# esologic/GANce

Measured on AMD Instinct MI355X. Metric: synthesized frames/sec at 1024x1024 config-f, higher is better.
Workload: dtype f32 (bf16x3 split operands, 6 terms, fp32 accumulate)

## Files before the change

### gance_amd/csrc/engine.hip

```cpp

#include <hip/hip_runtime.h>

#include <algorithm>
#include <cmath>
#include <cstdio>
#include <cstdlib>
#include <cstring>
#include <map>
#include <memory>
#include <mutex>
#include <string>
#include <tuple>
#include <vector>

#include "../../include/gance_hip.h"
#include "kernels.h"

namespace {

thread_local std::string g_last_error;

int fail(int code, const std::string& message) {
    g_last_error = message;
    return code;
// ... 218 lines not shown
    std::vector<size_t> wino64_w;
    float* noise_rand = nullptr;
    std::vector<size_t> noise_rand_off;
    int noise_rand_count = 0;
    bool noise_randomized = false;
    std::vector<size_t> wino43_w;
    std::vector<size_t> upfir_w;
    std::vector<size_t> upfir16_w;
    std::vector<size_t> winogemm_w;
    std::vector<size_t> upgemm_w;
    size_t up_packed_floats = 0, up_prod_floats = 0;
    int gemm_bf16 = 0;
    std::vector<size_t> upfir16x_w;
    std::vector<size_t> upfirs_w;
    int upfir_split = 1;
    int upfir_split_max_res = 1024;
    int num_cus = 256;
    std::vector<float> conv_ns;
    std::vector<int> conv_s_off, conv_d_off;
    std::vector<size_t> rgb_w, rgb_bias;
    std::vector<int> rgb_s_off;
    int ctot = 0, dtot = 0;
    int* blk_row = nullptr;
    gance::DemodLayer* demod_layers = nullptr;

    std::shared_ptr<gance_workspace> ws;
    std::map<std::tuple<int, int, unsigned, int, int>, GraphEntry> graphs;
    std::vector<int> t_units;
    size_t slab_floats = 0, y_floats = 0, rgb_part_floats = 0;

// ... 290 lines not shown
        if (form.wino43) form.wino64 = false;
        return form;
    };
    enum class UpFused { no, fp32, split };
    auto up_runs_fused = [&](int idx, gance::UpFirArgs* plan) -> UpFused {
        const ConvLayerHost& c = e->convs[idx];
        const int H = (1 << c.res_log2) / 2;
        static const int upfir_env = [] { const char* v = std::getenv("GANCE_TUNE_UPFIR"); return v ? std::atoi(v) : -1; }();
        const int upfir_mode = upfir_env >= 0 ? upfir_env
                                              : ((e->cfg.flags & GANCE_FLAG_SPLIT_UPFIR) ? 0 : ((e->cfg.flags & GANCE_FLAG_FORCE_FUSED_UPFIR) ? 2 : 1));
        if (!c.up || upfir_mode == 0 || (e->upfir_w[idx] == SIZE_MAX && e->upfir16_w[idx] == SIZE_MAX)) return UpFused::no;
        gance::UpFirArgs u{};
        u.Cin = c.cin;
        if (e->upfirs_w[idx] != SIZE_MAX && upfir_mode != 0) {
            gance::upfirs_plan(B, c.cout, H, H, e->num_cus, &u);
            if (e->upfir_split == 2 || (u.total_blocks >= e->num_cus * 9 / 16 && 2 * H <= e->upfir_split_max_res)) {
                if (plan != nullptr) *plan = u;
                return UpFused::split;
            }
            u = gance::UpFirArgs{};
            u.Cin = c.cin;
        }
        if (e->upfir16_w[idx] != SIZE_MAX)
            gance::upfir16_plan(B, c.cout, H, H, e->num_cus, &u);
        else
            gance::upfir_plan(B, c.cout, H, H, e->num_cus, &u);
        const int steps_per_seg = u.rows_per_seg / u.step_rows;
        if (plan != nullptr) *plan = u;
        return (upfir_mode == 2 || (u.total_blocks >= e->num_cus * 3 / 4 && (u.segs == 1 || steps_per_seg >= 4))) ? UpFused::fp32 : UpFused::no;
    };
    static const bool prescale_up = [] { const char* v = std::getenv("GANCE_TUNE_PRESCALE_UP"); return !(v && std::atoi(v) == 0); }();
// ... 386 lines not shown
    if (config->device < 0 || config->device >= device_count)
        return fail(GANCE_ERR_INVALID_ARGUMENT, "device ordinal out of range");
    gance::DeviceGuard guard(config->device);
    GANCE_HIP_CHECK(guard.status());
    int num_cus = 0;
    GANCE_HIP_CHECK(hipDeviceGetAttribute(&num_cus, hipDeviceAttributeMultiprocessorCount, config->device));

    gance_engine* e = new gance_engine();
    {
        const char* v = std::getenv("GANCE_TUNE_GEMM_BF16X6");
        e->gemm_bf16 = v != nullptr && std::atoi(v) != 0 ? 1 : 0;
        const char* const split = std::getenv("GANCE_TUNE_UPFIR_SPLIT");
        e->upfir_split = split != nullptr ? std::max(0, std::min(2, std::atoi(split))) : 1;
        const char* const split_res = std::getenv("GANCE_TUNE_UPFIR_SPLIT_MAXRES");
        if (split_res != nullptr) e->upfir_split_max_res = std::atoi(split_res);
    }
    e->cfg = *config;
    e->num_cus = num_cus > 0 ? num_cus : 256;
    e->res_log2 = res_log2;
    e->num_rows = res_log2 * 2 - 2;
    build_spec(res_log2, &e->convs, &e->rgbs);
    const int nconv = (int)e->convs.size();
    const int nrgb = (int)e->rgbs.size();

    e->conv_s_off.resize(nconv);
    e->conv_d_off.resize(nconv);
    e->rgb_s_off.resize(nrgb);
    int ctot = 0, dtot = 0;
    for (int i = 0; i < nconv; ++i) {
        e->conv_s_off[i] = ctot;
// ... 115 lines not shown
            const int split_mode = c.cout % 256 == 0 ? e->gemm_bf16 : 0;
            e->winogemm_w[i] = reserve(gance::winogemm_weight_floats(c.cin, c.cout) * (split_mode ? 3 : 2) / 2);
            if (split_mode) gance::winogemm_arrange_weights_split(scaled.data(), c.cin, c.cout, &pool[e->winogemm_w[i]]);
            else gance::winogemm_arrange_weights(scaled.data(), c.cin, c.cout, &pool[e->winogemm_w[i]]);
        }
        e->upgemm_w.push_back(SIZE_MAX);
        if (c.up && upgemm_min_columns() > 0 && gance::upgemm_supported(c.cin, c.cout, (1 << c.res_log2) / 2, (1 << c.res_log2) / 2)) {
            std::vector<float> scaled(wn);
            for (size_t j = 0; j < wn; ++j) scaled[j] = src[j] * coef;
            const int split_mode = (9 * c.cout) % 256 == 0 ? e->gemm_bf16 : 0;
            e->upgemm_w[i] = reserve(gance::upgemm_weight_floats(c.cin, c.cout) * (split_mode ? 3 : 2) / 2);
            if (split_mode) gance::upgemm_arrange_weights_split(scaled.data(), c.cin, c.cout, kUpTapWeight, &pool[e->upgemm_w[i]]);
            else gance::upgemm_arrange_weights(scaled.data(), c.cin, c.cout, kUpTapWeight, &pool[e->upgemm_w[i]]);
        }
        e->upfirs_w.push_back(SIZE_MAX);
        if (c.up && e->upfir_split != 0 && upfir16_mode() != 0 && gance::upfirs_supported(c.cin, c.cout, (1 << c.res_log2) / 2, (1 << c.res_log2) / 2)) {
            std::vector<float> scaled(wn);
            for (size_t j = 0; j < wn; ++j) scaled[j] = src[j] * coef;
            e->upfirs_w[i] = reserve(gance::upfirs_weight_floats(c.cin, c.cout));
            gance::upfirs_arrange_weights(scaled.data(), c.cin, c.cout, kUpTapWeight, &pool[e->upfirs_w[i]]);
        }
        e->upfir16x_w.push_back(SIZE_MAX);
        if (c.up && upfir16_mode() != 0 && upfir16x_mode() != 0 && gance::upfir16x_supported(c.cin, c.cout, (1 << c.res_log2) / 2, (1 << c.res_log2) / 2)) {
            std::vector<float> scaled(wn);
            for (size_t j = 0; j < wn; ++j) scaled[j] = src[j] * coef;
            e->upfir16x_w[i] = reserve(gance::upfir16x_weight_floats(c.cin, c.cout));
            gance::upfir16x_arrange_weights(scaled.data(), c.cin, c.cout, kUpTapWeight, &pool[e->upfir16x_w[i]]);
        }
        src += wn;
        demod_layers[i] = {(long long)w2_cursor, e->conv_s_off[i], e->conv_d_off[i], c.cin, c.cout};
        w2_cursor += (size_t)c.cin * c.cout;
// ... 386 lines not shown
```

### gance_amd/csrc/kernels.h

```cpp
#ifndef GANCE_KERNELS_H
#define GANCE_KERNELS_H

#include <hip/hip_runtime.h>
#include <stddef.h>
#include <stdint.h>

#include <mutex>
#include <string>

namespace gance {

class DeviceGuard {
  public:
    explicit DeviceGuard(int device) {
        if (hipGetDevice(&previous_) != hipSuccess) previous_ = -1;
        status_ = (device >= 0 && device != previous_) ? hipSetDevice(device) : hipSuccess;
        switched_ = status_ == hipSuccess && device >= 0 && device != previous_;
    }
    ~DeviceGuard() {
        if (switched_ && previous_ >= 0) (void)hipSetDevice(previous_);
    }
    DeviceGuard(const DeviceGuard&) = delete;
    DeviceGuard& operator=(const DeviceGuard&) = delete;
    hipError_t status() const { return status_; }
// ... 134 lines not shown
size_t upfir_weight_floats(int cin, int cout);
void upfir_arrange_weights(const float* w_in , int cin, int cout, const int* up_tap_weight, float* w_out);
void upfir_plan(int B, int cout, int H, int W, int num_cus, UpFirArgs* args);
hipError_t launch_upfir_fused(const UpFirArgs& args, hipStream_t stream);

bool upfir16_supported(int cin, int cout, int H, int W);
size_t upfir16_weight_floats(int cin, int cout);
void upfir16_arrange_weights(const float* w_in , int cin, int cout, const int* up_tap_weight, float* w_out);
void upfir16_plan(int B, int cout, int H, int W, int num_cus, UpFirArgs* args);
hipError_t launch_upfir16_fused(const UpFirArgs& args, hipStream_t stream);
bool upfir16x_supported(int cin, int cout, int H, int W);
size_t upfir16x_weight_floats(int cin, int cout);
void upfir16x_arrange_weights(const float* w_in , int cin, int cout, const int* up_tap_weight, float* w_out);

bool upfirs_supported(int cin, int cout, int H, int W);
size_t upfirs_weight_floats(int cin, int cout);
void upfirs_arrange_weights(const float* w_in , int cin, int cout, const int* up_tap_weight, float* w_out);
void upfirs_plan(int B, int cout, int H, int W, int num_cus, UpFirArgs* args);
hipError_t launch_upfir_split(const UpFirArgs& args, hipStream_t stream);

struct UpGemmArgs {
    const float* x;
    const float* w;
    const float* s;
    const float* d;
    float* packed;
    float* prod;
    float* t;
    long long x_b_stride, cls_stride, unit_stride;
    int B, Cin, Cout, H, W, s_stride, d_stride;
// ... 100 lines not shown
```

### gance_amd/csrc/upfir_split.hip

```cpp

#include <hip/hip_runtime.h>

#include <algorithm>
#include <cstdlib>
#include <cstring>
#include <type_traits>

#include "kernels.h"

#ifndef GANCE_UPFIRS_ABLATE
#define GANCE_UPFIRS_ABLATE 0
#endif

namespace gance {

namespace {

typedef float f32x4 __attribute__((ext_vector_type(4)));
typedef float f32x2 __attribute__((ext_vector_type(2)));
typedef unsigned u32x4 __attribute__((ext_vector_type(4)));
typedef __bf16 bf16x8 __attribute__((ext_vector_type(8)));
typedef __bf16 bf16x2 __attribute__((ext_vector_type(2)));
typedef __attribute__((address_space(3))) void* lds_ptr_t;

constexpr int kBM = 16;
constexpr int kKC = 32;
constexpr int kSW = 64;
constexpr int kTH = 8;
constexpr int kRows = kTH + 1;
constexpr int kPlanes = 12;
constexpr int kPlaneStride = 80;
constexpr int kSlotUnits = kPlanes * kPlaneStride;
constexpr int kRing = 3;
constexpr int kHaloCols = 4;
constexpr int kHaloUnits = kRows * kHaloCols * kPlanes;
constexpr int kHaloTasks = kRows * kHaloCols * 4;
#ifndef GANCE_UPFIRS_WEAVE
#define GANCE_UPFIRS_WEAVE 2
#endif
#ifndef GANCE_UPFIRS_MIN_SEG_ROWS
#define GANCE_UPFIRS_MIN_SEG_ROWS 16
#endif
#ifndef GANCE_UPFIRS_DEPTH
#define GANCE_UPFIRS_DEPTH 6
#endif
constexpr int kDepth = GANCE_UPFIRS_DEPTH;
constexpr int kCarryRows = 3;
constexpr int kPassCh = 4;
constexpr int kPassRows = 8;
constexpr int kTW = 2 * kSW + 4;
constexpr int kCG = kSW / 2;
constexpr int kRG = 64 / kCG;
constexpr int kFR = kPassRows / kRG;
constexpr int kWin = kFR + 3;
constexpr int kCarryFloats = kBM * kCarryRows * kTW;
constexpr int kStageFloats = kPassCh * kPassRows * kTW;
constexpr int kNzPieces = 2 * kPassRows * 2 * kSW / 256;
constexpr float kSqrt2f = 1.4142135623730951f;
static_assert((2 * kRows) % kDepth == 0 && kDepth + 2 < kRows && kRows % kRing == 0, "ring slots and staging registers rotate with the unrolled rows of a chunk pair");

constexpr size_t kRingBytes = (size_t)kRing * kSlotUnits * 16;
constexpr size_t kHaloBytes = (size_t)2 * kHaloUnits * 16;
constexpr int kWUnits = 27 * 64;
constexpr size_t kWBytes = (size_t)kWUnits * 16;
constexpr size_t lds_bytes(int cin) {
    return kRingBytes + kHaloBytes + kWBytes + sizeof(float) * ((size_t)kStageFloats + kNzPieces * 256 + kCarryFloats + cin + 3 * kBM);
}

__host__ __device__ constexpr int tap_cls(int t) { return t < 4 ? 0 : (t < 6 ? 1 : (t < 8 ? 2 : 3)); }
__host__ __device__ constexpr int tap_dy(int t) { return (t == 2 || t == 3 || t == 5) ? 1 : 0; }
__host__ __device__ constexpr int tap_dx(int t) { return (t == 1 || t == 3 || t == 7) ? 1 : 0; }

__device__ __forceinline__ void lds_barrier() {
    asm volatile("s_waitcnt lgkmcnt(0)" ::: "memory");
    __builtin_amdgcn_s_barrier();
    asm volatile("" ::: "memory");
}

__device__ __forceinline__ int fresh_lane() {
    int l;
    asm volatile("v_mbcnt_lo_u32_b32 %0, -1, 0\n\tv_mbcnt_hi_u32_b32 %0, -1, %0" : "=v"(l));
// ... 17 lines not shown
__device__ __forceinline__ void split_unit(const unsigned (&raw)[8], u32x4 (&part)[3]) {
    unsigned w[3][4];
    if (GANCE_UPFIRS_ABLATE & 1) {
#pragma unroll
        for (int q = 0; q < 3; ++q) part[q] = u32x4{raw[q], raw[q + 1], raw[q + 2], raw[q + 3]};
        return;
    }
#pragma unroll
    for (int e = 0; e < 4; ++e) split_pair(__builtin_bit_cast(float, raw[2 * e]), __builtin_bit_cast(float, raw[2 * e + 1]), w[0][e], w[1][e], w[2][e]);
#pragma unroll
    for (int q = 0; q < 3; ++q) part[q] = u32x4{w[q][0], w[q][1], w[q][2], w[q][3]};
}

}

template <bool kPre, bool kNoise>
__device__ __forceinline__ void upfirs_body(const UpFirArgs& p) {
    extern __shared__ __attribute__((aligned(16))) unsigned char smem_raw[];
    u32x4* const ring = reinterpret_cast<u32x4*>(smem_raw);
    u32x4* const halo = ring + kRing * kSlotUnits;
    u32x4* const w_lds = halo + 2 * kHaloUnits;
    float* const stage = reinterpret_cast<float*>(w_lds + kWUnits);
    float* const nz_lds = stage + kStageFloats;
    float* const carry = nz_lds + kNzPieces * 256;
    float* const s_lds = carry + kCarryFloats;
    float* const d_lds = s_lds + (kPre ? 0 : p.Cin);
    float* const b_lds = d_lds + kBM;
    float* const sn_lds = b_lds + kBM;

    const int tid = threadIdx.x;
    const int wave = __builtin_amdgcn_readfirstlane(tid >> 6);
    const int lane = tid & 63;
    const int n16 = lane & 15, kg = lane >> 4;

    int id;
    {
        const int v = blockIdx.x, nwg = p.total_blocks;
        const int q = nwg >> 3, r = nwg & 7, xcd = v & 7;
        id = (xcd < r ? xcd * (q + 1) : r * (q + 1) + (xcd - r) * q) + (v >> 3);
    }
    const int m_tile = id % p.m_tiles;
    id /= p.m_tiles;
    const int strip = id % p.strips;
    id /= p.strips;
    const int seg = id % p.segs;
    const int b = id / p.segs;
    const int m0 = m_tile * kBM;
    const int X0 = strip * kSW;
    const int H = p.H, W = p.W;
    const int Hp = H + 2, Wp = W + 8;
    const int HpWp4 = Hp * Wp * 4;
    const int chunks = p.Cin / kKC;
    const int steps = H / kTH;
    const int s_begin = seg * (p.rows_per_seg / kTH), s_end = s_begin + p.rows_per_seg / kTH;
    const int s_first = seg > 0 ? s_begin - 1 : s_begin;

    const __amdgpu_buffer_rsrc_t x_rsrc =
        __builtin_amdgcn_make_buffer_rsrc((void*)(p.x + (size_t)b * p.x_b_stride), 0, p.Cin * Hp * Wp * 4, 0x00020000);
    const __amdgpu_buffer_rsrc_t w_rsrc = __builtin_amdgcn_make_buffer_rsrc(
        (void*)(reinterpret_cast<const unsigned char*>(p.w) + (size_t)m_tile * chunks * 27 * 1024), 0, chunks * 27 * 1024, 0x00020000);

    const int st_pair = lane >> 4, st_g = lane & 15;
    u32x4* const ring_w = ring + wave * kPlaneStride + ring_column(4 * st_g + st_pair);
    const int m_pos = 16 * wave + n16;
    const u32x4* const ring_r0 = ring + kg * kPlaneStride + ring_column(m_pos);
    const u32x4* const ring_r1 = ring + kg * kPlaneStride + (m_pos > 0 ? ring_column(m_pos - 1) : kEdgeColumn);
    const bool edge_copy = wave == 3 && lane < kPlanes;
    const int e_unit = lane % kPlanes;
    u32x4* const ring_e = ring + (e_unit >> 2) * 4 * kPlaneStride + (e_unit & 3) * kPlaneStride + (edge_copy ? kEdgeColumn : 66 + wave);
    const u32x4* const halo_e = halo + e_unit;
    const u32x4* const halo_r = halo + ((n16 & 7) * kHaloCols + 2 * (n16 >> 3)) * kPlanes + kg;
    const u32x4* const halo_f = halo + ((kRows - 1) * kHaloCols + 2 * (n16 >> 3)) * kPlanes + kg;
    const int st_voff = (2 * st_pair * Hp * Wp + X0 + 4 + 4 * st_g) * 4;
    unsigned st[kDepth][8];
    auto stage_load = [&](unsigned(&dst)[8], int chunk, int brow, bool in_loop = false) {
        if ((GANCE_UPFIRS_ABLATE & 4) && in_loop) return;
        const int soff = ((chunk * kKC + wave * 8) * Hp + brow) * Wp * 4;
#pragma unroll
        for (int e = 0; e < 2; ++e) {
            const u32x4 q4 = __builtin_amdgcn_raw_buffer_load_b128(x_rsrc, st_voff, soff + e * HpWp4, 0);
#pragma unroll
            for (int c = 0; c < 4; ++c) dst[2 * c + e] = q4[c];
        }
    };
    auto scale_pair = [&](unsigned(&raw)[8], int chunk) {
        if constexpr (!kPre) {
            const f32x2 s2 = *reinterpret_cast<const f32x2*>(s_lds + chunk * kKC + 8 * wave + 2 * st_pair);
#pragma unroll
            for (int c = 0; c < 4; ++c) {
                raw[2 * c] = __builtin_bit_cast(unsigned, __builtin_bit_cast(float, raw[2 * c]) * s2[0]);
                raw[2 * c + 1] = __builtin_bit_cast(unsigned, __builtin_bit_cast(float, raw[2 * c + 1]) * s2[1]);
            }
        }
    };
    auto transpose_rows = [](u32x4& u) {
        auto a02 = __builtin_amdgcn_permlane32_swap(u[0], u[2], false, false);
        auto a13 = __builtin_amdgcn_permlane32_swap(u[1], u[3], false, false);
        auto b01 = __builtin_amdgcn_permlane16_swap(a02[0], a13[0], false, false);
        auto b23 = __builtin_amdgcn_permlane16_swap(a02[1], a13[1], false, false);
        u = u32x4{b01[0], b01[1], b23[0], b23[1]};
    };
    auto scale8 = [&](unsigned(&raw)[8], int chunk, int group) {
        if constexpr (!kPre) {
            const f32x4 s0 = *reinterpret_cast<const f32x4*>(s_lds + chunk * kKC + group * 8);
            const f32x4 s1 = *reinterpret_cast<const f32x4*>(s_lds + chunk * kKC + group * 8 + 4);
#pragma unroll
            for (int e = 0; e < 4; ++e) {
                raw[e] = __builtin_bit_cast(unsigned, __builtin_bit_cast(float, raw[e]) * s0[e]);
                raw[4 + e] = __builtin_bit_cast(unsigned, __builtin_bit_cast(float, raw[4 + e]) * s1[e]);
            }
        }
    };
    auto stage_store = [&](unsigned(&raw)[8], int slot, int chunk) {
        scale_pair(raw, chunk);
        u32x4 part[3];
        split_unit(raw, part);
#pragma unroll
        for (int q = 0; q < 3; ++q) transpose_rows(part[q]);
#pragma unroll
        for (int q = 0; q < 3; ++q)
            if (!(GANCE_UPFIRS_ABLATE & 16)) ring_w[slot * kSlotUnits + q * 4 * kPlaneStride] = part[q];
    };
    auto edge_store = [&](int slot, int hbuf, int hrow) { if (!(GANCE_UPFIRS_ABLATE & 64)) ring_e[slot * kSlotUnits] = halo_e[hbuf * kHaloUnits + (hrow * kHaloCols + 1) * kPlanes]; };
    const int h_task = tid < kHaloTasks ? tid : tid - kHaloTasks;
    const int h_col = h_task & 3, h_kg = (h_task >> 2) & 3, h_row = h_task >> 4;
    const int h_voff = ((h_kg * 8 * Hp + h_row) * Wp + X0 + 2 + (h_col & 1) + (h_col >> 1) * 65) * 4;
    u32x4* const halo_w = halo + (h_row * kHaloCols + h_col) * kPlanes + h_kg;
    unsigned hraw[8];
    auto halo_load = [&](int step, int chunk) {
        const int soff = (chunk * kKC * Hp + kTH * step) * Wp * 4;
#pragma unroll
        for (int e = 0; e < 8; ++e) hraw[e] = __builtin_amdgcn_raw_buffer_load_b32(x_rsrc, h_voff, soff + e * HpWp4, 0);
    };
    auto halo_store = [&](int chunk, int buf) {
        scale8(hraw, chunk, h_kg);
        u32x4 part[3];
        split_unit(hraw, part);
#pragma unroll
        for (int q = 0; q < 3; ++q) halo_w[buf * kHaloUnits + q * 4] = part[q];
    };

// ... 18 lines not shown
    u32x4 Bf[2][2][3];
    auto load_b = [&](int slot, u32x4(&dst)[2][3]) {
#pragma unroll
        for (int q = 0; q < 3; ++q) {
            dst[0][q] = ring_r0[slot * kSlotUnits + q * 4 * kPlaneStride];
            dst[1][q] = ring_r1[slot * kSlotUnits + q * 4 * kPlaneStride];
        }
    };

    stage_load(st[0], 0, kTH * s_first + 0);
    stage_load(st[1], 0, kTH * s_first + 1);
    load_a3(0, 0, A[0]);
    halo_load(s_first, 0);
    if constexpr (!kPre)
        for (int i = tid; i < p.Cin; i += 256) s_lds[i] = p.s[(size_t)b * p.s_stride + i];
    if (tid < kBM) {
        d_lds[tid] = p.d[(size_t)b * p.d_stride + m0 + tid];
        b_lds[tid] = p.bias[m0 + tid];
        sn_lds[tid] = p.s_next != nullptr ? p.s_next[(size_t)b * p.s_stride + m0 + tid] : 1.0f;
    }
    for (int i = tid; i < kCarryFloats; i += 256) carry[i] = 0.f;
#pragma unroll
    for (int t = 1; t < 9; ++t) load_a3(0, t, A[t]);
    if constexpr (!kPre) lds_barrier();
    stage_store(st[0], 0, 0);
    stage_store(st[1], 1, 0);
    halo_store(0, 0);
#pragma unroll
    for (int r = 2; r < 2 + kDepth; ++r) stage_load(st[r % kDepth], 0, kTH * s_first + r);
    lds_barrier();
    edge_store(0, 0, 0);
    edge_store(1, 0, 1);
    lds_barrier();
    load_b(0, Bf[0]);

    const int OW = 2 * W, OWp = OW + 8;
// ... 6 lines not shown

    constexpr int kTerms[6][2] = {{2, 0}, {0, 2}, {1, 1}, {1, 0}, {0, 1}, {0, 0}};
    constexpr int kTapTurn[9] = {0, 4, 6, 8, 2, 5, 1, 7, 3};

#pragma unroll 1
    for (int si = s_first; si < s_end; ++si) {
        const int y0 = kTH * si;
        const bool last_step = si + 1 == steps;
        const bool priming = si < s_begin;
        f32x4 acc[kTH][4];
#pragma unroll
        for (int r = 0; r < kTH; ++r)
#pragma unroll
            for (int c = 0; c < 4; ++c) acc[r][c] = f32x4{0.f, 0.f, 0.f, 0.f};
        f32x4 accf[2] = {f32x4{0.f, 0.f, 0.f, 0.f}, f32x4{0.f, 0.f, 0.f, 0.f}};
        f32x4 acch = f32x4{0.f, 0.f, 0.f, 0.f}, acchf = f32x4{0.f, 0.f, 0.f, 0.f};

        auto run_chunk = [&](auto parity, const int chunk) {
            constexpr int ab = decltype(parity)::value;
            const int n_chunk = chunk + 1 < chunks ? chunk + 1 : 0;
            const int n_step = chunk + 1 < chunks ? si : (last_step ? si : si + 1);
#pragma unroll
            for (int j = 0; j < kRows; ++j) {
                const int cur = (j + ab) & 1;
                if (j == 0) weights_dma(n_chunk);
                if (j == 0) halo_load(n_step, n_chunk);
                if (j == 4) halo_store(n_chunk, ab ^ 1);
                load_b((j + 1) % kRing, Bf[cur ^ 1]);
                edge_store((j + 2) % kRing, j + 2 < kRows ? ab : ab ^ 1, (j + 2) % kRows);
                stage_store(st[(kRows * ab + j + 2) % kDepth], (j + 2) % kRing, j + 2 < kRows ? chunk : n_chunk);
                stage_load(st[(kRows * ab + j + 2) % kDepth], j + 2 + kDepth < kRows ? chunk : n_chunk, kTH * (j + 2 + kDepth < kRows ? si : n_step) + (j + 2 + kDepth) % kRows, true);
                if (j + 1 < kRows) {
#pragma unroll
                    for (int term = 0; term < ((GANCE_UPFIRS_ABLATE & 8) ? 0 : 6); ++term)
#pragma unroll
                        for (int k = 0; k < 9; ++k) {
                            const int t = kTapTurn[k];
                            const int row = tap_dy(t) ? j : j - 1;
                            if (row < 0 || row >= kTH) continue;
                            acc[row][tap_cls(t)] = __builtin_amdgcn_mfma_f32_16x16x32_bf16(
// ... 12 lines not shown
                    for (int i = 0; i < 9; ++i) {
                        const int t = kOrder[i];
                        if (!tap_dy(t)) {
#pragma unroll
                            for (int term = 0; term < 6; ++term)
                                acc[kTH - 1][tap_cls(t)] = __builtin_amdgcn_mfma_f32_16x16x32_bf16(
                                    __builtin_bit_cast(bf16x8, A[t][kTerms[term][1]]), __builtin_bit_cast(bf16x8, Bf[cur][tap_dx(t)][kTerms[term][0]]),
                                    acc[kTH - 1][tap_cls(t)], 0, 0, 0);
                        } else if (last_step) {
#pragma unroll
                            for (int term = 0; term < 6; ++term)
                                accf[tap_cls(t)] = __builtin_amdgcn_mfma_f32_16x16x32_bf16(
                                    __builtin_bit_cast(bf16x8, A[t][kTerms[term][1]]), __builtin_bit_cast(bf16x8, Bf[cur][tap_dx(t)][kTerms[term][0]]),
                                    accf[tap_cls(t)], 0, 0, 0);
                        }
                        if (wave == tap_cls(t) && !(GANCE_UPFIRS_ABLATE & 64)) {
                            u32x4 hf[3];
#pragma unroll
                            for (int q = 0; q < 3; ++q) hf[q] = halo_r[ab * kHaloUnits + ((1 - tap_dy(t)) * kHaloCols + 1 - tap_dx(t)) * kPlanes + q * 4];
#pragma unroll
                            for (int term = 0; term < 6; ++term)
                                acch = __builtin_amdgcn_mfma_f32_16x16x32_bf16(__builtin_bit_cast(bf16x8, A[t][kTerms[term][1]]),
                                                                               __builtin_bit_cast(bf16x8, hf[kTerms[term][0]]), acch, 0, 0, 0);
                            if (last_step && tap_dy(t)) {
#pragma unroll
                                for (int q = 0; q < 3; ++q) hf[q] = halo_f[ab * kHaloUnits + (1 - tap_dx(t)) * kPlanes + q * 4];
#pragma unroll
                                for (int term = 0; term < 6; ++term)
                                    acchf = __builtin_amdgcn_mfma_f32_16x16x32_bf16(__builtin_bit_cast(bf16x8, A[t][kTerms[term][1]]),
                                                                                    __builtin_bit_cast(bf16x8, hf[kTerms[term][0]]), acchf, 0, 0, 0);
                            }
                        }
                        read_a3(t, A[t]);
                    }
                }
                if (j == kRows - 2) asm volatile("s_waitcnt vmcnt(24)" ::: "memory");
                if (!(GANCE_UPFIRS_ABLATE & 32)) lds_barrier();
            }
        };
#pragma unroll 1
        for (int chunk = 0; chunk < chunks; chunk += 2) {
            run_chunk(std::integral_constant<int, 0>{}, chunk);
            run_chunk(std::integral_constant<int, 1>{}, chunk + 1);
        }

        const int elane = fresh_lane();
        const int en16 = elane & 15, eq4 = elane >> 4;
        const int dump_base = eq4 * (kPassRows * kTW) + 32 * wave + 2 * en16 + 1;
        const int hpy = wave >> 1, hpx = wave & 1;
        const int fc = wave;
        const int cg = elane % kCG;
        const int rg = elane / kCG;
        const int o_voff = (int)((fc * oplane + (long long)(kFR * rg) * OWp + 4 * cg) * 4);

        auto run_passes = [&](auto flush_tag) {
            constexpr bool kFlush = decltype(flush_tag)::value;
            const int ys = kFlush ? H : y0;
            if (kNoise) {
#pragma unroll
                for (int i = 0; i < kNzPieces / 4; ++i) {
                    const int f = (wave + 4 * i) * 256 + 4 * elane;
                    const int row = f / (2 * kSW), col = f % (2 * kSW);
                    __builtin_amdgcn_raw_ptr_buffer_load_lds(nz_rsrc, (lds_ptr_t)(nz_lds + (wave + 4 * i) * 256), 16,
                                                             ((2 * ys - 2 + row) * OW + 2 * X0 + col) * 4, 0, 0, 0);
                }
                asm volatile("s_waitcnt vmcnt(0)" ::: "memory");
            }
            constexpr int kRowPasses = kFlush ? 1 : 2;
#pragma unroll
            for (int rw = 0; rw < kRowPasses; ++rw) {
                const int oy0 = 2 * (ys + 4 * rw) - 2;
                const int r_lo = max(0, -oy0);
                const int r_hi = priming ? 0 : min(kPassRows, 2 * H - oy0);
#pragma unroll
                for (int g = 0; g < 4; ++g) {
                    if constexpr (kFlush) {
#pragma unroll
                        for (int c = 0; c < 4; ++c) stage[dump_base + (c >> 1) * kTW + (c & 1)] = c < 2 ? accf[c][g] : 0.f;
                        if (en16 == 0 || en16 == 8) {
                            const int side = en16 >> 3;
                            if (hpy == 0 && (side == 1 || hpx == 1)) stage[eq4 * (kPassRows * kTW) + (side ? 2 * kSW + 1 + hpx : 0)] = acchf[g];
                            if (hpy == 1 && (side == 1 || hpx == 1)) stage[eq4 * (kPassRows * kTW) + kTW + (side ? 2 * kSW + 1 + hpx : 0)] = 0.f;
                        }
                    } else {
#pragma unroll
                        for (int r4 = 0; r4 < 4; ++r4)
#pragma unroll
                            for (int c = 0; c < 4; ++c) stage[dump_base + (2 * r4 + (c >> 1)) * kTW + (c & 1)] = acc[4 * rw + r4][c][g];
                        const int row = en16 & 7, side = en16 >> 3;
                        if ((side == 1 || hpx == 1) && row / 4 == rw)
                            stage[eq4 * (kPassRows * kTW) + (2 * (row % 4) + hpy) * kTW + (side ? 2 * kSW + 1 + hpx : 0)] = acch[g];
                    }
                    lds_barrier();

                    const int ch = 4 * g + fc;
                    const float dsc = d_lds[ch] * kSqrt2f;
                    const float kh0 = 0.25f * dsc, kh1 = 0.75f * dsc;
                    const float bias2 = b_lds[ch] * kSqrt2f;
                    const float lr6 = 0.6f * sn_lds[ch], lr4 = 0.4f * sn_lds[ch];
                    const float* const win_lo = carry + ch * (kCarryRows * kTW) + (kFR * rg) * kTW + 4 * cg;
                    const float* const win_hi = stage + fc * (kPassRows * kTW) + (kFR * rg - kCarryRows) * kTW + 4 * cg;
                    f32x4 ta[kWin], tb[kWin];
#pragma unroll
                    for (int i = 0; i < kWin; ++i) {
                        const float* const rowp = (i < kCarryRows && kFR * rg + i < kCarryRows ? win_lo : win_hi) + i * kTW;
                        ta[i] = *reinterpret_cast<const f32x4*>(rowp);
                        tb[i] = *reinterpret_cast<const f32x4*>(rowp + 4);
                    }
                    {
                        const int o_soff = (int)((4 * g * oplane + (long long)(oy0 + 3) * OWp + 2 * X0 + 4) * 4);
// ... 20 lines not shown
                        }
                    }
                    lds_barrier();
                    if (!kFlush && rg == kRG - 1) {
                        float* const carry_w = carry + ch * (kCarryRows * kTW) + 4 * cg;
#pragma unroll
                        for (int i = 0; i < 3; ++i) {
                            *reinterpret_cast<f32x4*>(carry_w + i * kTW) = ta[kWin - 3 + i];
                            if (cg == kCG - 1) *reinterpret_cast<f32x4*>(carry_w + i * kTW + 4) = tb[kWin - 3 + i];
                        }
                    }
                }
            }
        };
        if (GANCE_UPFIRS_ABLATE & 2) {
            float sum = acch[0] + acchf[0] + accf[0][0] + accf[1][0];
#pragma unroll
            for (int r = 0; r < kTH; ++r)
#pragma unroll
                for (int c = 0; c < 4; ++c) sum += acc[r][c][0] + acc[r][c][3];
            if (sum == 12345.678f) p.out[tid] = sum;
            continue;
        }
        run_passes(std::false_type{});
        if (last_step) {
            lds_barrier();
            run_passes(std::true_type{});
        }
    }
}

bool upfirs_supported(int cin, int cout, int H, int W) {
    return H == W && W % kSW == 0 && H % kTH == 0 && cin % (2 * kKC) == 0 && cout % kBM == 0 && cin <= 512;
}

size_t upfirs_weight_floats(int cin, int cout) { return (size_t)(cout / kBM) * (cin / kKC) * 27 * 256; }

static unsigned short bf16_rne_host(float x) {
    unsigned u;
    std::memcpy(&u, &x, 4);
    u += 0x7fffu + ((u >> 16) & 1u);
    return (unsigned short)(u >> 16);
}
static float bf16_value_host(unsigned short h) {
    const unsigned u = (unsigned)h << 16;
    float f;
    std::memcpy(&f, &u, 4);
    return f;
// ... 8 lines not shown
                for (int k = 0; k < kKC; ++k)
                    for (int m = 0; m < kBM; ++m) {
                        const int channel = 4 * (m & 3) + (m >> 2);
                        const float v = w_in[((size_t)up_tap_weight[t] * cin + ch * kKC + k) * cout + mt * kBM + channel];
                        unsigned short part[3];
                        part[0] = bf16_rne_host(v);
                        const float r1 = v - bf16_value_host(part[0]);
                        part[1] = bf16_rne_host(r1);
                        part[2] = bf16_rne_host(r1 - bf16_value_host(part[1]));
                        for (int q = 0; q < 3; ++q)
                            out[((((((size_t)mt * chunks + ch) * 9 + t) * 3 + q) * 4 + k / 8) * 16 + m) * 8 + k % 8] = part[q];
                    }
}

void upfirs_plan(int B, int cout, int H, int W, int num_cus, UpFirArgs* a) {
    a->m_tiles = cout / kBM;
    a->strips = W / kSW;
    a->step_rows = kTH;
    static const bool segments = [] { const char* v = std::getenv("GANCE_TUNE_UPFIR_SPLIT_SEGS"); return !(v && std::atoi(v) == 0); }();
    int segs = 1;
    const int base = B * a->m_tiles * a->strips;
    long long best = (long long)((base + num_cus - 1) / num_cus) * H;
    for (int n = 2; segments && H / n >= GANCE_UPFIRS_MIN_SEG_ROWS && (H / n) % kTH == 0 && base * (n / 2) < num_cus; n *= 2) {
        const long long cost = (long long)((base * n + num_cus - 1) / num_cus) * (H / n + kTH);
        if (cost < best) best = cost, segs = n;
    }
    a->segs = segs;
    a->rows_per_seg = H / segs;
    a->total_blocks = base * segs;
    a->stagger_phases = 1;
    a->stagger_ticks = 0;
    a->debug_flags = 0;
}

__global__ __launch_bounds__(256, 1) void upfirs_fused_kernel(const UpFirArgs p) { upfirs_body<false, false>(p); }
__global__ __launch_bounds__(256, 1) void upfirs_fused_noise_kernel(const UpFirArgs p) { upfirs_body<false, true>(p); }
__global__ __launch_bounds__(256, 1) void upfirs_fused_pre_kernel(const UpFirArgs p) { upfirs_body<true, false>(p); }
__global__ __launch_bounds__(256, 1) void upfirs_fused_pre_noise_kernel(const UpFirArgs p) { upfirs_body<true, true>(p); }

hipError_t launch_upfir_split(const UpFirArgs& args, hipStream_t stream) {
    using Kernel = void (*)(const UpFirArgs);
    static const Kernel kernels[4] = {upfirs_fused_kernel, upfirs_fused_noise_kernel, upfirs_fused_pre_kernel, upfirs_fused_pre_noise_kernel};
    static PerDeviceInt ready;
    int unused = 0;
    const hipError_t e = ready.get(
        [&](int, int* value) {
            *value = 1;
            for (int i = 0; i < 4; ++i) {
                const hipError_t err =
                    hipFuncSetAttribute(reinterpret_cast<const void*>(kernels[i]), hipFuncAttributeMaxDynamicSharedMemorySize, (int)lds_bytes(i >= 2 ? 0 : 512));
                if (err != hipSuccess) return err;
            }
            return hipSuccess;
        },
        &unused);
    if (e != hipSuccess) return e;
    if (!upfirs_supported(args.Cin, args.Cout, args.H, args.W) || args.segs < 1 || args.rows_per_seg * args.segs != args.H || args.rows_per_seg % kTH != 0 ||
        args.total_blocks != args.B * args.m_tiles * args.strips * args.segs)
        return hipErrorInvalidValue;
    const int pre = args.input_prescaled ? 1 : 0, noise = args.noise != nullptr ? 1 : 0;
    hipLaunchKernelGGL(kernels[2 * pre + noise], dim3(args.total_blocks), dim3(256), lds_bytes(pre ? 0 : args.Cin), stream, args);
    return hipGetLastError();
}

}
```

Measured before the change: 1417.

## Add narrow-width variants of split upfir kernel for 16 and 32 wide layers

Templates the split-operand fused upsample+FIR conv kernel on a tile count NT so that layers narrower than the 64-wide strip (16x16 and 32x32 outputs) can use it. Each block covers several output-channel tiles instead of one wide strip. Weights are loaded directly from global memory rather than via the LDS weight DMA, and halo handling is adapted. The goal is to replace the slower fp32 or unfused path at low resolutions, at the cost of more kernel variants and weight loads from global memory.

New measurement: 1464 (median of 6 runs). +3.3%, better.

```diff
diff --git a/gance_amd/csrc/engine.hip b/gance_amd/csrc/engine.hip
--- a/gance_amd/csrc/engine.hip
+++ b/gance_amd/csrc/engine.hip
@@ -256,6 +256,7 @@
     std::vector<size_t> upfir16x_w;
     std::vector<size_t> upfirs_w;
     int upfir_split = 1;
+    int upfir_split_narrow = 1;
     int upfir_split_max_res = 1024;
     int num_cus = 256;
     std::vector<float> conv_ns;
@@ -576,7 +577,8 @@
         u.Cin = c.cin;
         if (e->upfirs_w[idx] != SIZE_MAX && upfir_mode != 0) {
             gance::upfirs_plan(B, c.cout, H, H, e->num_cus, &u);
-            if (e->upfir_split == 2 || (u.total_blocks >= e->num_cus * 9 / 16 && 2 * H <= e->upfir_split_max_res)) {
+            const bool narrow = !gance::upfirs_supported(c.cin, c.cout, H, H);
+            if ((e->upfir_split == 2 && !narrow) || (u.total_blocks >= e->num_cus * 9 / 16 && 2 * H <= e->upfir_split_max_res)) {
                 if (plan != nullptr) *plan = u;
                 return UpFused::split;
             }
@@ -993,6 +995,8 @@
         e->upfir_split = split != nullptr ? std::max(0, std::min(2, std::atoi(split))) : 1;
         const char* const split_res = std::getenv("GANCE_TUNE_UPFIR_SPLIT_MAXRES");
         if (split_res != nullptr) e->upfir_split_max_res = std::atoi(split_res);
+        const char* const split_narrow = std::getenv("GANCE_TUNE_UPFIR_SPLIT_NARROW");
+        e->upfir_split_narrow = split_narrow != nullptr && std::atoi(split_narrow) == 0 ? 0 : 1;
     }
     e->cfg = *config;
     e->num_cus = num_cus > 0 ? num_cus : 256;
@@ -1138,7 +1142,9 @@
             else gance::upgemm_arrange_weights(scaled.data(), c.cin, c.cout, kUpTapWeight, &pool[e->upgemm_w[i]]);
         }
         e->upfirs_w.push_back(SIZE_MAX);
-        if (c.up && e->upfir_split != 0 && upfir16_mode() != 0 && gance::upfirs_supported(c.cin, c.cout, (1 << c.res_log2) / 2, (1 << c.res_log2) / 2)) {
+        if (c.up && e->upfir_split != 0 && upfir16_mode() != 0 &&
+            (gance::upfirs_supported(c.cin, c.cout, (1 << c.res_log2) / 2, (1 << c.res_log2) / 2) ||
+             (e->upfir_split_narrow != 0 && gance::upfirs_narrow_supported(c.cin, c.cout, (1 << c.res_log2) / 2, (1 << c.res_log2) / 2)))) {
             std::vector<float> scaled(wn);
             for (size_t j = 0; j < wn; ++j) scaled[j] = src[j] * coef;
             e->upfirs_w[i] = reserve(gance::upfirs_weight_floats(c.cin, c.cout));
diff --git a/gance_amd/csrc/kernels.h b/gance_amd/csrc/kernels.h
--- a/gance_amd/csrc/kernels.h
+++ b/gance_amd/csrc/kernels.h
@@ -172,6 +172,7 @@
 void upfir16x_arrange_weights(const float* w_in , int cin, int cout, const int* up_tap_weight, float* w_out);
 
 bool upfirs_supported(int cin, int cout, int H, int W);
+bool upfirs_narrow_supported(int cin, int cout, int H, int W);
 size_t upfirs_weight_floats(int cin, int cout);
 void upfirs_arrange_weights(const float* w_in , int cin, int cout, const int* up_tap_weight, float* w_out);
 void upfirs_plan(int B, int cout, int H, int W, int num_cus, UpFirArgs* args);
diff --git a/gance_amd/csrc/upfir_split.hip b/gance_amd/csrc/upfir_split.hip
--- a/gance_amd/csrc/upfir_split.hip
+++ b/gance_amd/csrc/upfir_split.hip
@@ -19,6 +19,7 @@
 typedef float f32x4 __attribute__((ext_vector_type(4)));
 typedef float f32x2 __attribute__((ext_vector_type(2)));
 typedef unsigned u32x4 __attribute__((ext_vector_type(4)));
+typedef unsigned u32x2 __attribute__((ext_vector_type(2)));
 typedef __bf16 bf16x8 __attribute__((ext_vector_type(8)));
 typedef __bf16 bf16x2 __attribute__((ext_vector_type(2)));
 typedef __attribute__((address_space(3))) void* lds_ptr_t;
@@ -48,23 +49,33 @@
 constexpr int kCarryRows = 3;
 constexpr int kPassCh = 4;
 constexpr int kPassRows = 8;
-constexpr int kTW = 2 * kSW + 4;
-constexpr int kCG = kSW / 2;
-constexpr int kRG = 64 / kCG;
-constexpr int kFR = kPassRows / kRG;
-constexpr int kWin = kFR + 3;
-constexpr int kCarryFloats = kBM * kCarryRows * kTW;
-constexpr int kStageFloats = kPassCh * kPassRows * kTW;
-constexpr int kNzPieces = 2 * kPassRows * 2 * kSW / 256;
 constexpr float kSqrt2f = 1.4142135623730951f;
 static_assert((2 * kRows) % kDepth == 0 && kDepth + 2 < kRows && kRows % kRing == 0, "ring slots and staging registers rotate with the unrolled rows of a chunk pair");
 
+template <int NT>
+struct Geo {
+    static constexpr int kSW = 64 / NT;
+    static constexpr int kBMB = kBM * NT;
+    static constexpr int kTC = kSW / 16;
+    static constexpr int kPW = 4 / NT;
+    static constexpr int kTW = 2 * kSW + 4;
+    static constexpr int kCG = kSW / 2;
+    static constexpr int kRG = 64 / NT / kCG;
+    static constexpr int kFR = kPassRows / kRG;
+    static constexpr int kWin = kFR + 3;
+    static constexpr int kCarryFloats = kBMB * kCarryRows * kTW;
+    static constexpr int kStageFloats = kPassCh * NT * kPassRows * kTW;
+    static constexpr int kNzPieces = 2 * kPassRows * 2 * kSW / 256;
+    static constexpr int kWUnits = NT == 1 ? 27 * 64 : 0;
+};
+
 constexpr size_t kRingBytes = (size_t)kRing * kSlotUnits * 16;
 constexpr size_t kHaloBytes = (size_t)2 * kHaloUnits * 16;
-constexpr int kWUnits = 27 * 64;
-constexpr size_t kWBytes = (size_t)kWUnits * 16;
+template <int NT>
 constexpr size_t lds_bytes(int cin) {
-    return kRingBytes + kHaloBytes + kWBytes + sizeof(float) * ((size_t)kStageFloats + kNzPieces * 256 + kCarryFloats + cin + 3 * kBM);
+    using G = Geo<NT>;
+    return kRingBytes + kHaloBytes + (size_t)G::kWUnits * 16 +
+           sizeof(float) * ((size_t)G::kStageFloats + G::kNzPieces * 256 + G::kCarryFloats + cin + 3 * G::kBMB);
 }
 
 __host__ __device__ constexpr int tap_cls(int t) { return t < 4 ? 0 : (t < 6 ? 1 : (t < 8 ? 2 : 3)); }
@@ -112,24 +123,28 @@
 
 }
 
-template <bool kPre, bool kNoise>
+template <int NT, bool kPre, bool kNoise>
 __device__ __forceinline__ void upfirs_body(const UpFirArgs& p) {
+    using G = Geo<NT>;
+    constexpr int kSW = G::kSW, kBMB = G::kBMB, kTC = G::kTC, kPW = G::kPW, kTW = G::kTW, kCG = G::kCG, kRG = G::kRG, kFR = G::kFR,
+                  kWin = G::kWin, kCarryFloats = G::kCarryFloats, kStageFloats = G::kStageFloats, kNzPieces = G::kNzPieces;
     extern __shared__ __attribute__((aligned(16))) unsigned char smem_raw[];
     u32x4* const ring = reinterpret_cast<u32x4*>(smem_raw);
     u32x4* const halo = ring + kRing * kSlotUnits;
     u32x4* const w_lds = halo + 2 * kHaloUnits;
-    float* const stage = reinterpret_cast<float*>(w_lds + kWUnits);
+    float* const stage = reinterpret_cast<float*>(w_lds + G::kWUnits);
     float* const nz_lds = stage + kStageFloats;
     float* const carry = nz_lds + kNzPieces * 256;
     float* const s_lds = carry + kCarryFloats;
     float* const d_lds = s_lds + (kPre ? 0 : p.Cin);
-    float* const b_lds = d_lds + kBM;
-    float* const sn_lds = b_lds + kBM;
+    float* const b_lds = d_lds + kBMB;
+    float* const sn_lds = b_lds + kBMB;
 
     const int tid = threadIdx.x;
     const int wave = __builtin_amdgcn_readfirstlane(tid >> 6);
     const int lane = tid & 63;
     const int n16 = lane & 15, kg = lane >> 4;
+    const int ct = NT == 1 ? 0 : wave / kTC, tc = NT == 1 ? wave : wave % kTC;
 
     int id;
     {
@@ -143,7 +158,7 @@
     id /= p.strips;
     const int seg = id % p.segs;
     const int b = id / p.segs;
-    const int m0 = m_tile * kBM;
+    const int m0 = m_tile * kBMB;
     const int X0 = strip * kSW;
     const int H = p.H, W = p.W;
     const int Hp = H + 2, Wp = W + 8;
@@ -156,11 +171,13 @@
     const __amdgpu_buffer_rsrc_t x_rsrc =
         __builtin_amdgcn_make_buffer_rsrc((void*)(p.x + (size_t)b * p.x_b_stride), 0, p.Cin * Hp * Wp * 4, 0x00020000);
     const __amdgpu_buffer_rsrc_t w_rsrc = __builtin_amdgcn_make_buffer_rsrc(
-        (void*)(reinterpret_cast<const unsigned char*>(p.w) + (size_t)m_tile * chunks * 27 * 1024), 0, chunks * 27 * 1024, 0x00020000);
+        (void*)(reinterpret_cast<const unsigned char*>(p.w) + (size_t)(m_tile * NT + ct) * chunks * 27 * 1024), 0, chunks * 27 * 1024, 0x00020000);
 
     const int st_pair = lane >> 4, st_g = lane & 15;
     u32x4* const ring_w = ring + wave * kPlaneStride + ring_column(4 * st_g + st_pair);
-    const int m_pos = 16 * wave + n16;
+    unsigned* const ring_wn = reinterpret_cast<unsigned*>(ring + wave * kPlaneStride + ring_column(NT == 2 ? 2 * st_g + (st_pair & 1) : st_g)) +
+                              (NT == 2 ? 2 * (st_pair >> 1) : st_pair);
+    const int m_pos = 16 * tc + n16;
     const u32x4* const ring_r0 = ring + kg * kPlaneStride + ring_column(m_pos);
     const u32x4* const ring_r1 = ring + kg * kPlaneStride + (m_pos > 0 ? ring_column(m_pos - 1) : kEdgeColumn);
     const bool edge_copy = wave == 3 && lane < kPlanes;
@@ -169,23 +186,31 @@
     const u32x4* const halo_e = halo + e_unit;
     const u32x4* const halo_r = halo + ((n16 & 7) * kHaloCols + 2 * (n16 >> 3)) * kPlanes + kg;
     const u32x4* const halo_f = halo + ((kRows - 1) * kHaloCols + 2 * (n16 >> 3)) * kPlanes + kg;
-    const int st_voff = (2 * st_pair * Hp * Wp + X0 + 4 + 4 * st_g) * 4;
+    const int st_voff = (2 * st_pair * Hp * Wp + X0 + 4 + kPW * st_g) * 4;
     unsigned st[kDepth][8];
     auto stage_load = [&](unsigned(&dst)[8], int chunk, int brow, bool in_loop = false) {
         if ((GANCE_UPFIRS_ABLATE & 4) && in_loop) return;
         const int soff = ((chunk * kKC + wave * 8) * Hp + brow) * Wp * 4;
 #pragma unroll
         for (int e = 0; e < 2; ++e) {
-            const u32x4 q4 = __builtin_amdgcn_raw_buffer_load_b128(x_rsrc, st_voff, soff + e * HpWp4, 0);
-#pragma unroll
-            for (int c = 0; c < 4; ++c) dst[2 * c + e] = q4[c];
+            if constexpr (kPW == 4) {
+                const u32x4 q4 = __builtin_amdgcn_raw_buffer_load_b128(x_rsrc, st_voff, soff + e * HpWp4, 0);
+#pragma unroll
+                for (int c = 0; c < 4; ++c) dst[2 * c + e] = q4[c];
+            } else if constexpr (kPW == 2) {
+                const u32x2 q2 = __builtin_amdgcn_raw_buffer_load_b64(x_rsrc, st_voff, soff + e * HpWp4, 0);
+                dst[e] = q2[0];
+                dst[2 + e] = q2[1];
+            } else {
+                dst[e] = __builtin_amdgcn_raw_buffer_load_b32(x_rsrc, st_voff, soff + e * HpWp4, 0);
+            }
         }
     };
     auto scale_pair = [&](unsigned(&raw)[8], int chunk) {
         if constexpr (!kPre) {
             const f32x2 s2 = *reinterpret_cast<const f32x2*>(s_lds + chunk * kKC + 8 * wave + 2 * st_pair);
 #pragma unroll
-            for (int c = 0; c < 4; ++c) {
+            for (int c = 0; c < kPW; ++c) {
                 raw[2 * c] = __builtin_bit_cast(unsigned, __builtin_bit_cast(float, raw[2 * c]) * s2[0]);
                 raw[2 * c + 1] = __builtin_bit_cast(unsigned, __builtin_bit_cast(float, raw[2 * c + 1]) * s2[1]);
             }
@@ -211,18 +236,34 @@
     };
     auto stage_store = [&](unsigned(&raw)[8], int slot, int chunk) {
         scale_pair(raw, chunk);
-        u32x4 part[3];
-        split_unit(raw, part);
-#pragma unroll
-        for (int q = 0; q < 3; ++q) transpose_rows(part[q]);
-#pragma unroll
-        for (int q = 0; q < 3; ++q)
-            if (!(GANCE_UPFIRS_ABLATE & 16)) ring_w[slot * kSlotUnits + q * 4 * kPlaneStride] = part[q];
+        if constexpr (NT == 1) {
+            u32x4 part[3];
+            split_unit(raw, part);
+#pragma unroll
+            for (int q = 0; q < 3; ++q) transpose_rows(part[q]);
+#pragma unroll
+            for (int q = 0; q < 3; ++q)
+                if (!(GANCE_UPFIRS_ABLATE & 16)) ring_w[slot * kSlotUnits + q * 4 * kPlaneStride] = part[q];
+        } else {
+            unsigned w[3][kPW];
+#pragma unroll
+            for (int c = 0; c < kPW; ++c) split_pair(__builtin_bit_cast(float, raw[2 * c]), __builtin_bit_cast(float, raw[2 * c + 1]), w[0][c], w[1][c], w[2][c]);
+#pragma unroll
+            for (int q = 0; q < 3; ++q) {
+                unsigned* const dst = ring_wn + 4 * (slot * kSlotUnits + q * 4 * kPlaneStride);
+                if constexpr (NT == 2) {
+                    const auto s = __builtin_amdgcn_permlane16_swap(w[q][0], w[q][1], false, false);
+                    *reinterpret_cast<u32x2*>(dst) = u32x2{s[0], s[1]};
+                } else {
+                    *dst = w[q][0];
+                }
+            }
+        }
     };
     auto edge_store = [&](int slot, int hbuf, int hrow) { if (!(GANCE_UPFIRS_ABLATE & 64)) ring_e[slot * kSlotUnits] = halo_e[hbuf * kHaloUnits + (hrow * kHaloCols + 1) * kPlanes]; };
     const int h_task = tid < kHaloTasks ? tid : tid - kHaloTasks;
     const int h_col = h_task & 3, h_kg = (h_task >> 2) & 3, h_row = h_task >> 4;
-    const int h_voff = ((h_kg * 8 * Hp + h_row) * Wp + X0 + 2 + (h_col & 1) + (h_col >> 1) * 65) * 4;
+    const int h_voff = ((h_kg * 8 * Hp + h_row) * Wp + X0 + 2 + (h_col & 1) + (h_col >> 1) * (kSW + 1)) * 4;
     u32x4* const halo_w = halo + (h_row * kHaloCols + h_col) * kPlanes + h_kg;
     unsigned hraw[8];
     auto halo_load = [&](int step, int chunk) {
@@ -271,12 +312,14 @@
     halo_load(s_first, 0);
     if constexpr (!kPre)
         for (int i = tid; i < p.Cin; i += 256) s_lds[i] = p.s[(size_t)b * p.s_stride + i];
-    if (tid < kBM) {
+    if (tid < kBMB) {
         d_lds[tid] = p.d[(size_t)b * p.d_stride + m0 + tid];
         b_lds[tid] = p.bias[m0 + tid];
         sn_lds[tid] = p.s_next != nullptr ? p.s_next[(size_t)b * p.s_stride + m0 + tid] : 1.0f;
     }
     for (int i = tid; i < kCarryFloats; i += 256) carry[i] = 0.f;
+    if constexpr (NT > 1)
+        for (int i = tid; i < kPassCh * NT * kPassRows; i += 256) stage[i * kTW] = stage[i * kTW + 2 * kSW + 2] = stage[i * kTW + 2 * kSW + 3] = 0.f;
 #pragma unroll
     for (int t = 1; t < 9; ++t) load_a3(0, t, A[t]);
     if constexpr (!kPre) lds_barrier();
@@ -313,7 +356,7 @@
 #pragma unroll
             for (int c = 0; c < 4; ++c) acc[r][c] = f32x4{0.f, 0.f, 0.f, 0.f};
         f32x4 accf[2] = {f32x4{0.f, 0.f, 0.f, 0.f}, f32x4{0.f, 0.f, 0.f, 0.f}};
-        f32x4 acch = f32x4{0.f, 0.f, 0.f, 0.f}, acchf = f32x4{0.f, 0.f, 0.f, 0.f};
+        f32x4 acch[NT == 1 ? 1 : 2] = {}, acchf = f32x4{0.f, 0.f, 0.f, 0.f};
 
         auto run_chunk = [&](auto parity, const int chunk) {
             constexpr int ab = decltype(parity)::value;
@@ -322,7 +365,7 @@
 #pragma unroll
             for (int j = 0; j < kRows; ++j) {
                 const int cur = (j + ab) & 1;
-                if (j == 0) weights_dma(n_chunk);
+                if (NT == 1 && j == 0) weights_dma(n_chunk);
                 if (j == 0) halo_load(n_step, n_chunk);
                 if (j == 4) halo_store(n_chunk, ab ^ 1);
                 load_b((j + 1) % kRing, Bf[cur ^ 1]);
@@ -365,14 +408,16 @@
                                     __builtin_bit_cast(bf16x8, A[t][kTerms[term][1]]), __builtin_bit_cast(bf16x8, Bf[cur][tap_dx(t)][kTerms[term][0]]),
                                     accf[tap_cls(t)], 0, 0, 0);
                         }
-                        if (wave == tap_cls(t) && !(GANCE_UPFIRS_ABLATE & 64)) {
+                        const int hc = NT == 1 ? 0 : tap_cls(t) >> 1;
+                        const bool halo_mine = NT == 1 ? wave == tap_cls(t) : (tap_dx(t) && (tap_cls(t) & 1) == 0 && (kTC == 1 || tc == hc));
+                        if (halo_mine && !(GANCE_UPFIRS_ABLATE & 64)) {
                             u32x4 hf[3];
 #pragma unroll
                             for (int q = 0; q < 3; ++q) hf[q] = halo_r[ab * kHaloUnits + ((1 - tap_dy(t)) * kHaloCols + 1 - tap_dx(t)) * kPlanes + q * 4];
 #pragma unroll
                             for (int term = 0; term < 6; ++term)
-                                acch = __builtin_amdgcn_mfma_f32_16x16x32_bf16(__builtin_bit_cast(bf16x8, A[t][kTerms[term][1]]),
-                                                                               __builtin_bit_cast(bf16x8, hf[kTerms[term][0]]), acch, 0, 0, 0);
+                                acch[hc] = __builtin_amdgcn_mfma_f32_16x16x32_bf16(__builtin_bit_cast(bf16x8, A[t][kTerms[term][1]]),
+                                                                                    __builtin_bit_cast(bf16x8, hf[kTerms[term][0]]), acch[hc], 0, 0, 0);
                             if (last_step && tap_dy(t)) {
 #pragma unroll
                                 for (int q = 0; q < 3; ++q) hf[q] = halo_f[ab * kHaloUnits + (1 - tap_dx(t)) * kPlanes + q * 4];
@@ -382,10 +427,11 @@
                                                                                     __builtin_bit_cast(bf16x8, hf[kTerms[term][0]]), acchf, 0, 0, 0);
                             }
                         }
-                        read_a3(t, A[t]);
+                        if constexpr (NT == 1) read_a3(t, A[t]);
+                        else load_a3(n_chunk, t, A[t]);
                     }
                 }
-                if (j == kRows - 2) asm volatile("s_waitcnt vmcnt(24)" ::: "memory");
+                if (NT == 1 && j == kRows - 2) asm volatile("s_waitcnt vmcnt(24)" ::: "memory");
                 if (!(GANCE_UPFIRS_ABLATE & 32)) lds_barrier();
             }
         };
@@ -397,19 +443,22 @@
 
         const int elane = fresh_lane();
         const int en16 = elane & 15, eq4 = elane >> 4;
-        const int dump_base = eq4 * (kPassRows * kTW) + 32 * wave + 2 * en16 + 1;
+        const int dump_base = (4 * ct + eq4) * (kPassRows * kTW) + 32 * tc + 2 * en16 + 1;
         const int hpy = wave >> 1, hpx = wave & 1;
-        const int fc = wave;
-        const int cg = elane % kCG;
-        const int rg = elane / kCG;
-        const int o_voff = (int)((fc * oplane + (long long)(kFR * rg) * OWp + 4 * cg) * 4);
+        const int fsub = NT == 1 ? 0 : elane / (64 / NT), flane = NT == 1 ? elane : elane % (64 / NT);
+        const int fc = NT == 1 ? wave : wave * NT + fsub;
+        const int fch = NT == 1 ? fc : 16 * (fc >> 2) + (fc & 3);
+        const int cg = flane % kCG;
+        const int rg = flane / kCG;
+        const int o_voff = (int)((fch * oplane + (long long)(kFR * rg) * OWp + 4 * cg) * 4);
 
         auto run_passes = [&](auto flush_tag) {
             constexpr bool kFlush = decltype(flush_tag)::value;
             const int ys = kFlush ? H : y0;
             if (kNoise) {
 #pragma unroll
-                for (int i = 0; i < kNzPieces / 4; ++i) {
+                for (int i = 0; i < (kNzPieces + 3) / 4; ++i) {
+                    if (kNzPieces % 4 != 0 && wave + 4 * i >= kNzPieces) break;
                     const int f = (wave + 4 * i) * 256 + 4 * elane;
                     const int row = f / (2 * kSW), col = f % (2 * kSW);
                     __builtin_amdgcn_raw_ptr_buffer_load_lds(nz_rsrc, (lds_ptr_t)(nz_lds + (wave + 4 * i) * 256), 16,
@@ -428,10 +477,15 @@
                     if constexpr (kFlush) {
 #pragma unroll
                         for (int c = 0; c < 4; ++c) stage[dump_base + (c >> 1) * kTW + (c & 1)] = c < 2 ? accf[c][g] : 0.f;
-                        if (en16 == 0 || en16 == 8) {
-                            const int side = en16 >> 3;
-                            if (hpy == 0 && (side == 1 || hpx == 1)) stage[eq4 * (kPassRows * kTW) + (side ? 2 * kSW + 1 + hpx : 0)] = acchf[g];
-                            if (hpy == 1 && (side == 1 || hpx == 1)) stage[eq4 * (kPassRows * kTW) + kTW + (side ? 2 * kSW + 1 + hpx : 0)] = 0.f;
+                        if constexpr (NT == 1) {
+                            if (en16 == 0 || en16 == 8) {
+                                const int side = en16 >> 3;
+                                if (hpy == 0 && (side == 1 || hpx == 1)) stage[eq4 * (kPassRows * kTW) + (side ? 2 * kSW + 1 + hpx : 0)] = acchf[g];
+                                if (hpy == 1 && (side == 1 || hpx == 1)) stage[eq4 * (kPassRows * kTW) + kTW + (side ? 2 * kSW + 1 + hpx : 0)] = 0.f;
+                            }
+                        } else if (en16 == 8 && tc == 0) {
+                            stage[(4 * ct + eq4) * (kPassRows * kTW) + 2 * kSW + 1] = acchf[g];
+                            stage[(4 * ct + eq4) * (kPassRows * kTW) + kTW + 2 * kSW + 1] = 0.f;
                         }
                     } else {
 #pragma unroll
@@ -439,12 +493,18 @@
 #pragma unroll
                             for (int c = 0; c < 4; ++c) stage[dump_base + (2 * r4 + (c >> 1)) * kTW + (c & 1)] = acc[4 * rw + r4][c][g];
                         const int row = en16 & 7, side = en16 >> 3;
-                        if ((side == 1 || hpx == 1) && row / 4 == rw)
-                            stage[eq4 * (kPassRows * kTW) + (2 * (row % 4) + hpy) * kTW + (side ? 2 * kSW + 1 + hpx : 0)] = acch[g];
+                        if constexpr (NT == 1) {
+                            if ((side == 1 || hpx == 1) && row / 4 == rw)
+                                stage[eq4 * (kPassRows * kTW) + (2 * (row % 4) + hpy) * kTW + (side ? 2 * kSW + 1 + hpx : 0)] = acch[0][g];
+                        } else if (side == 1 && row / 4 == rw) {
+#pragma unroll
+                            for (int h = 0; h < 2; ++h)
+                                if (kTC == 1 || tc == h) stage[(4 * ct + eq4) * (kPassRows * kTW) + (2 * (row % 4) + h) * kTW + 2 * kSW + 1] = acch[h][g];
+                        }
                     }
                     lds_barrier();
 
-                    const int ch = 4 * g + fc;
+                    const int ch = 4 * g + fch;
                     const float dsc = d_lds[ch] * kSqrt2f;
                     const float kh0 = 0.25f * dsc, kh1 = 0.75f * dsc;
                     const float bias2 = b_lds[ch] * kSqrt2f;
@@ -495,7 +555,7 @@
             }
         };
         if (GANCE_UPFIRS_ABLATE & 2) {
-            float sum = acch[0] + acchf[0] + accf[0][0] + accf[1][0];
+            float sum = acch[0][0] + acchf[0] + accf[0][0] + accf[1][0];
 #pragma unroll
             for (int r = 0; r < kTH; ++r)
 #pragma unroll
@@ -513,6 +573,10 @@
 
 bool upfirs_supported(int cin, int cout, int H, int W) {
     return H == W && W % kSW == 0 && H % kTH == 0 && cin % (2 * kKC) == 0 && cout % kBM == 0 && cin <= 512;
+}
+
+bool upfirs_narrow_supported(int cin, int cout, int H, int W) {
+    return H == W && (W == 32 || W == 16) && H % kTH == 0 && cin % (2 * kKC) == 0 && cout % (kBM * (kSW / W)) == 0 && cin <= 512;
 }
 
 size_t upfirs_weight_floats(int cin, int cout) { return (size_t)(cout / kBM) * (cin / kKC) * 27 * 256; }
@@ -551,9 +615,20 @@
 }
 
 void upfirs_plan(int B, int cout, int H, int W, int num_cus, UpFirArgs* a) {
+    a->step_rows = kTH;
+    a->stagger_phases = 1;
+    a->stagger_ticks = 0;
+    a->debug_flags = 0;
+    if (W < kSW) {
+        a->m_tiles = cout / (kBM * (kSW / W));
+        a->strips = 1;
+        a->segs = 1;
+        a->rows_per_seg = H;
+        a->total_blocks = B * a->m_tiles;
+        return;
+    }
     a->m_tiles = cout / kBM;
     a->strips = W / kSW;
-    a->step_rows = kTH;
     static const bool segments = [] { const char* v = std::getenv("GANCE_TUNE_UPFIR_SPLIT_SEGS"); return !(v && std::atoi(v) == 0); }();
     int segs = 1;
     const int base = B * a->m_tiles * a->strips;
@@ -565,38 +640,51 @@
     a->segs = segs;
     a->rows_per_seg = H / segs;
     a->total_blocks = base * segs;
-    a->stagger_phases = 1;
-    a->stagger_ticks = 0;
-    a->debug_flags = 0;
-}
-
-__global__ __launch_bounds__(256, 1) void upfirs_fused_kernel(const UpFirArgs p) { upfirs_body<false, false>(p); }
-__global__ __launch_bounds__(256, 1) void upfirs_fused_noise_kernel(const UpFirArgs p) { upfirs_body<false, true>(p); }
-__global__ __launch_bounds__(256, 1) void upfirs_fused_pre_kernel(const UpFirArgs p) { upfirs_body<true, false>(p); }
-__global__ __launch_bounds__(256, 1) void upfirs_fused_pre_noise_kernel(const UpFirArgs p) { upfirs_body<true, true>(p); }
+}
+
+__global__ __launch_bounds__(256, 1) void upfirs_fused_kernel(const UpFirArgs p) { upfirs_body<1, false, false>(p); }
+__global__ __launch_bounds__(256, 1) void upfirs_fused_noise_kernel(const UpFirArgs p) { upfirs_body<1, false, true>(p); }
+__global__ __launch_bounds__(256, 1) void upfirs_fused_pre_kernel(const UpFirArgs p) { upfirs_body<1, true, false>(p); }
+__global__ __launch_bounds__(256, 1) void upfirs_fused_pre_noise_kernel(const UpFirArgs p) { upfirs_body<1, true, true>(p); }
+__global__ __launch_bounds__(256, 1) void upfirs_w32_fused_kernel(const UpFirArgs p) { upfirs_body<2, false, false>(p); }
+__global__ __launch_bounds__(256, 1) void upfirs_w32_fused_noise_kernel(const UpFirArgs p) { upfirs_body<2, false, true>(p); }
+__global__ __launch_bounds__(256, 1) void upfirs_w32_fused_pre_kernel(const UpFirArgs p) { upfirs_body<2, true, false>(p); }
+__global__ __launch_bounds__(256, 1) void upfirs_w32_fused_pre_noise_kernel(const UpFirArgs p) { upfirs_body<2, true, true>(p); }
+__global__ __launch_bounds__(256, 1) void upfirs_w16_fused_kernel(const UpFirArgs p) { upfirs_body<4, false, false>(p); }
+__global__ __launch_bounds__(256, 1) void upfirs_w16_fused_noise_kernel(const UpFirArgs p) { upfirs_body<4, false, true>(p); }
+__global__ __launch_bounds__(256, 1) void upfirs_w16_fused_pre_kernel(const UpFirArgs p) { upfirs_body<4, true, false>(p); }
+__global__ __launch_bounds__(256, 1) void upfirs_w16_fused_pre_noise_kernel(const UpFirArgs p) { upfirs_body<4, true, true>(p); }
 
 hipError_t launch_upfir_split(const UpFirArgs& args, hipStream_t stream) {
     using Kernel = void (*)(const UpFirArgs);
-    static const Kernel kernels[4] = {upfirs_fused_kernel, upfirs_fused_noise_kernel, upfirs_fused_pre_kernel, upfirs_fused_pre_noise_kernel};
+    static const Kernel kernels[3][4] = {
+        {upfirs_fused_kernel, upfirs_fused_noise_kernel, upfirs_fused_pre_kernel, upfirs_fused_pre_noise_kernel},
+        {upfirs_w32_fused_kernel, upfirs_w32_fused_noise_kernel, upfirs_w32_fused_pre_kernel, upfirs_w32_fused_pre_noise_kernel},
+        {upfirs_w16_fused_kernel, upfirs_w16_fused_noise_kernel, upfirs_w16_fused_pre_kernel, upfirs_w16_fused_pre_noise_kernel}};
+    static size_t (*const lds_of[3])(int) = {lds_bytes<1>, lds_bytes<2>, lds_bytes<4>};
     static PerDeviceInt ready;
     int unused = 0;
     const hipError_t e = ready.get(
         [&](int, int* value) {
             *value = 1;
-            for (int i = 0; i < 4; ++i) {
-                const hipError_t err =
-                    hipFuncSetAttribute(reinterpret_cast<const void*>(kernels[i]), hipFuncAttributeMaxDynamicSharedMemorySize, (int)lds_bytes(i >= 2 ? 0 : 512));
-                if (err != hipSuccess) return err;
-            }
+            for (int gi = 0; gi < 3; ++gi)
+                for (int i = 0; i < 4; ++i) {
+                    const hipError_t err = hipFuncSetAttribute(reinterpret_cast<const void*>(kernels[gi][i]), hipFuncAttributeMaxDynamicSharedMemorySize,
+                                                               (int)lds_of[gi](i >= 2 ? 0 : 512));
+                    if (err != hipSuccess) return err;
+                }
             return hipSuccess;
         },
         &unused);
     if (e != hipSuccess) return e;
-    if (!upfirs_supported(args.Cin, args.Cout, args.H, args.W) || args.segs < 1 || args.rows_per_seg * args.segs != args.H || args.rows_per_seg % kTH != 0 ||
-        args.total_blocks != args.B * args.m_tiles * args.strips * args.segs)
+    const int gi = args.W % kSW == 0 ? 0 : (args.W == 32 ? 1 : 2);
+    const bool narrow = gi != 0;
+    if (!(narrow ? upfirs_narrow_supported(args.Cin, args.Cout, args.H, args.W) : upfirs_supported(args.Cin, args.Cout, args.H, args.W)) || args.segs < 1 ||
+        args.rows_per_seg * args.segs != args.H || args.rows_per_seg % kTH != 0 || args.total_blocks != args.B * args.m_tiles * args.strips * args.segs ||
+        (narrow && (args.segs != 1 || args.strips != 1 || args.m_tiles * kBM * (kSW / args.W) != args.Cout)))
         return hipErrorInvalidValue;
     const int pre = args.input_prescaled ? 1 : 0, noise = args.noise != nullptr ? 1 : 0;
-    hipLaunchKernelGGL(kernels[2 * pre + noise], dim3(args.total_blocks), dim3(256), lds_bytes(pre ? 0 : args.Cin), stream, args);
+    hipLaunchKernelGGL(kernels[gi][2 * pre + noise], dim3(args.total_blocks), dim3(256), lds_of[gi](pre ? 0 : args.Cin), stream, args);
     return hipGetLastError();
 }
 
```
